# hritikbharucha/Custom_Porechop_ABI

Measured on AMD Instinct MI355X. Metric: reads/sec trimmed (100k ONT reads x 50 adapter pairs), higher is better.
Workload: dtype int32

## Files before the change

custom_porechop_abi_amd/csrc/pcabi_dp.h:

```cpp
#pragma once

#ifndef PCABI_ROW_FENCE
#define PCABI_ROW_FENCE 1
#endif
#ifndef PCABI_TAB_PD
#define PCABI_TAB_PD 0
#endif
#ifndef PCABI_TAB_PD_LONG
#define PCABI_TAB_PD_LONG 1
#endif

#include <stdint.h>
#include <algorithm>

#ifdef __HIPCC__
#define PCABI_HD __host__ __device__ __forceinline__
#else
#define PCABI_HD inline
#endif

namespace pcabi {

constexpr int NEG = -(1 << 28);

// ... 892 lines not shown
PCABI_HD bool shift_ok(int L, int rpl, const Scoring &s, int &P, int &B) {
    for (int p = shift_pmax(rpl); p >= 2; p >>= 1) {
        int blo, bhi;
        if (shift_range(L, rpl, s, p, blo, bhi)) {
            P = p;
            B = (blo + bhi) / 2;
            return true;
        }
    }
    return false;
}

PCABI_HD bool packed_ok(int L, int rpl, const Scoring &s) {
    switch (rpl) {
#define PCABI_PK(R) case R: return packed_ok_t<R>(L, s);
    PCABI_PK(4) PCABI_PK(8) PCABI_PK(12) PCABI_PK(16) PCABI_PK(20) PCABI_PK(24) PCABI_PK(28) PCABI_PK(32)
    PCABI_PK(36) PCABI_PK(40) PCABI_PK(44) PCABI_PK(48) PCABI_PK(52) PCABI_PK(56) PCABI_PK(60) PCABI_PK(64)
    PCABI_PK(68) PCABI_PK(72) PCABI_PK(76) PCABI_PK(80) PCABI_PK(84) PCABI_PK(88)
#undef PCABI_PK
    default: return false;
    }
}

template <int RPL, bool AFFINE, typename LAY = pk::Lay<RPL>, int PD = PCABI_TAB_PD>
struct LanePacked {
    using Y = LAY;
    int32_t G[RPL + 1];
    int32_t HK[RPL + 1];
    int bscore, bi, bj, blt, btrail, bprec;
    uint32_t battr;
    int slt_last, ht_last, hp_last;
    int32_t k_ge, k_go, k_gev, k_geh, neg2;
    int32_t k_gex, k_vo;
    int32_t bkey;

    template <typename TabRow, bool LAST, bool GATE = false>
    PCABI_HD void column(const TabRow &tab, const int j, const int L, const int off, const bool owned = true) {
        int32_t gup = Y::start(j + off) + k_go;
        int32_t vup = neg2;
        int slt_up = LT_NONE, vt_up = 0, vp_up = 0;
        int32_t lv = 0, lh = 0, ls = 0;
        int lslt = LT_D;
        bool lhext = false;
        constexpr int NQ = RPL / 4;
        int32_t t[RPL + 2];
        if (PD > 0) {
// ... 388 lines not shown
    const int np = (n - 1) / 4;
    uint32_t cur = tr(0), nx = tr(1);
    int j = 1;
#pragma unroll 1
    for (int q = 0; q < np; ++q, j += 4) {
        const uint32_t w = cur;
        cur = nx;
        nx = tr(q + 2);
        ls.advance();
        ls.template column<decltype(tabfn(0))>(tabfn((int)(w & 0xFFu)), j, off);
        ls.step();
        ls.template column<decltype(tabfn(0))>(tabfn((int)((w >> 8) & 0xFFu)), j + 1, off);
        ls.step();
        ls.template column<decltype(tabfn(0))>(tabfn((int)((w >> 16) & 0xFFu)), j + 2, off);
        ls.step();
        ls.template column<decltype(tabfn(0))>(tabfn((int)(w >> 24)), j + 3, off);
    }
#pragma unroll 1
    for (; j < n; ++j) {
        ls.advance();
        ls.template column<decltype(tabfn(0))>(tabfn((int)((cur >> (8 * ((j - 1) & 3))) & 0xFFu)), j, off);
    }
    return shift_last<RPL, PD>(ls, tabfn((int)((cur >> (8 * ((n - 1) & 3))) & 0xFFu)), n, L, sc);
}

template <int RPL, bool AFFINE, bool CHUNK = false, typename ReadFn, typename TabFn0, typename TabFn1>
PCABI_HD Result align_lane_packed_long(ReadFn &rd0, ReadFn &rd1, int n, const TabFn0 &tab0, const TabFn1 &tab1,
                                       int L, const Scoring sc, int own_lo = 1, int own_hi = -1) {
    int n_fin;
    Best b = packed_best<RPL, AFFINE, CHUNK, pk::LayL<RPL, 0>, PCABI_TAB_PD_LONG>(rd0, n, tab0, L, sc, own_lo, own_hi,
                                                                                 n_fin);
    const Best bm = packed_best<RPL, AFFINE, CHUNK, pk::LayL<RPL, 1>, PCABI_TAB_PD_LONG>(rd1, n, tab1, L, sc, own_lo,
                                                                                        own_hi, n_fin);
    b.attr |= bm.attr;
    return finish(b, L, n_fin);
}

struct SplitIn {
    int32_t gup, vup;
    int slt, vt, vp;
    int score, bi, lt, trail, prec;
    uint32_t attr;
};

template <int R, bool AFFINE, typename LAY>
struct LaneSplit {
// ... 352 lines not shown
```

custom_porechop_abi_amd/csrc/pcabi_engine.hip:

```cpp
#include <hip/hip_runtime.h>

#include <algorithm>
#include <atomic>
#include <cstdio>
#include <cstdlib>
#include <cstring>
#include <mutex>
#include <string>
#include <thread>
#include <vector>

#include "../../include/pcabi.h"
#include "pcabi_dp.h"
#include "pcabi_kern.h"
#include "pcabi_host.h"

namespace {
thread_local std::string g_err;
}

namespace pcabi_eng {
int fail(int code, const std::string &msg) {
    g_err = msg;
    return code;
// ... 327 lines not shown
        dispatch_fast(d.rpl, d.kind == GENERIC, p, affine, grid, st);
    return 0;
}

bool bucket_packed_ok(int b, const std::vector<int32_t> &lens, const pcabi::Scoring &sc) {
    if (kBuckets[b].kind == WIDE || kBuckets[b].kind == LONG) return true;
    if (kBuckets[b].kind != FAST || kBuckets[b].rpl > pcabi::pk::MAX_RPL) return false;
    for (int32_t L : lens)
        if (!pcabi::packed_ok(L, kBuckets[b].rpl, sc)) return false;
    return true;
}

int bucket_pack_mode(int b, const std::vector<int32_t> &lens, const pcabi::Scoring &sc) {
    if (!bucket_packed_ok(b, lens, sc)) return 0;
    if (kBuckets[b].kind != FAST || kBuckets[b].rpl > 32) return 1;
    for (int32_t L : lens)
        if (!pcabi::layt_ok(L, kBuckets[b].rpl, sc)) return 1;
    return 2;
}


void bucket_shift(int b, const std::vector<int32_t> &lens, const pcabi::Scoring &sc, int pack_mode, KParams &p) {
    p.shift_p = p.shift_b = 0;
    if (pack_mode != 2 || lens.empty() || sc.go == sc.ge) return;
    const char *e = std::getenv("PCABI_SHIFT");
    if (e && e[0] == '0') return;
    const int rpl = kBuckets[b].rpl;
    for (int P = pcabi::shift_pmax(rpl); P >= 2; P >>= 1) {
        int lo = INT32_MIN, hi = INT32_MAX;
        bool ok = true;
        for (int32_t L : lens) {
            int blo, bhi;
            if (!pcabi::shift_range(L, rpl, sc, P, blo, bhi)) { ok = false; break; }
            lo = std::max(lo, blo);
            hi = std::min(hi, bhi);
        }
        if (ok && lo <= hi) {
            p.shift_p = P;
            p.shift_b = lo + (hi - lo) / 2;
            return;
        }
    }
}

}

namespace {

constexpr int kMaxFastBuckets = 4;

// ... 660 lines not shown
```

custom_porechop_abi_amd/csrc/pcabi_k_group.hip:

```cpp
#include "pcabi_kern.h"

namespace pcabi_eng {

template <int CLS>
__global__ __launch_bounds__(256) void k_align_group(GroupParams gp) {
    constexpr int MAXR = group_max_rpl(CLS);
    __shared__ __attribute__((aligned(16))) int32_t tab[4 * kTabW * MAXR];
    int32_t *wave_tab = tab + (threadIdx.x >> 6) * kTabW * MAXR;
    const int64_t b = blockIdx.x;
    int s = 0;
    while (s + 1 < gp.n_seg && b >= gp.seg[s + 1].block0) ++s;
    const GroupSeg &g = gp.seg[s];
    KParams p{};
    p.tiles = g.tiles;
    p.tile_off = g.tile_off;
    p.win_len = g.win_len;
    p.n_win = g.n_win;
    p.adp_pad = g.adp_pad;
    p.adp_len = g.adp_len;
    p.adp_id = g.adp_id;
    p.n_adp = g.n_adp;
    p.out = g.out;
    p.out_stride = g.out_stride;
    p.sc = gp.sc;
    p.shift_p = g.shift_p;
    p.shift_b = g.shift_b;
    const int64_t lb = b - g.block0;
    if constexpr (CLS == 0) {
        if (g.shift_p > 0) {
            switch (g.rpl) {
#define T(R) case R: cross_block<R, true, SHIFT>(p, lb, wave_tab); break;
            T(4) T(8) T(12) T(16) T(20) T(24) T(28) T(32)
#undef T
            }
        } else {
            switch (g.rpl) {
#define T(R) case R: cross_block<R, true, TAGGED>(p, lb, wave_tab); break;
            T(4) T(8) T(12) T(16) T(20) T(24) T(28) T(32)
#undef T
            }
        }
    } else {
        switch (g.rpl) {
#define P(R) case R: cross_block<R, true, PACKED>(p, lb, wave_tab); break;
        P(36) P(40) P(44) P(48) P(52) P(56) P(60) P(64)
#undef P
        }
    }
}

void dispatch_group(int cls, const GroupParams &p, int64_t blocks, hipStream_t st) {
    if (blocks <= 0) return;
    if (cls == 0) hipLaunchKernelGGL((k_align_group<0>), dim3((unsigned)blocks), dim3(256), 0, st, p);
    else hipLaunchKernelGGL((k_align_group<1>), dim3((unsigned)blocks), dim3(256), 0, st, p);
}

}
```

custom_porechop_abi_amd/csrc/pcabi_k_packed_large.hip:

```cpp
#include "pcabi_kern.h"

namespace pcabi_eng {

void dispatch_packed_large(int rpl, bool long_kind, const KParams &p, bool affine, dim3 grid, hipStream_t st) {
    if (long_kind) {
        switch (rpl) {
        case 96: launch<96, LONG>(p, affine, grid, st); break;
        case 112: launch<112, LONG>(p, affine, grid, st); break;
        case 128: launch<128, LONG>(p, affine, grid, st); break;
        }
        return;
    }
    switch (rpl) {
#define C(R) case R: launch<R, PACKED>(p, affine, grid, st); break;
    C(36) C(40) C(44) C(48) C(52) C(56) C(60) C(64) C(68) C(72) C(76) C(80) C(84) C(88)
#undef C
    }
}

}
```

custom_porechop_abi_amd/csrc/pcabi_kern.h:

```cpp
#pragma once
#include <hip/hip_runtime.h>

#include <algorithm>
#include <cstdint>
#include <cstdlib>
#include <string>
#include <type_traits>

#include "../../include/pcabi.h"
#include "pcabi_dp.h"

#ifndef PCABI_WAVES
#define PCABI_WAVES 1
#endif

void pcabi_poison(void *p, size_t bytes);
void pcabi_poison_async(void *p, size_t bytes, hipStream_t st);

namespace pcabi_eng {

int fail(int code, const std::string &msg);

#define HIP_TRY(expr)                                                                   \
    do {                                                                                \
        hipError_t e_ = (expr);                                                         \
        if (e_ != hipSuccess)                                                           \
            return fail(PCABI_E_DEVICE, std::string(#expr) + ": " + hipGetErrorString(e_)); \
    } while (0)

enum Kind { FAST = 0, GENERIC = 1, PACKED = 2, WIDE = 3, LONG = 4, STRIPED = 5,
            TAGGED = 6,
            SHIFT = 7 };
struct BucketDef {
    int rpl;
    Kind kind;
};
constexpr BucketDef kBuckets[] = {
    {4, FAST},  {8, FAST},  {12, FAST}, {16, FAST}, {20, FAST}, {24, FAST}, {28, FAST}, {32, FAST},
    {36, FAST}, {40, FAST}, {44, FAST}, {48, FAST}, {52, FAST}, {56, FAST}, {60, FAST}, {64, FAST},
    {68, WIDE}, {72, WIDE}, {76, WIDE}, {80, WIDE}, {84, WIDE}, {88, WIDE},
    {96, LONG}, {112, LONG}, {128, LONG},
    {16, GENERIC}, {32, GENERIC}, {64, GENERIC}, {96, GENERIC}, {128, GENERIC},
    {256, STRIPED}};
constexpr int kNumBuckets = sizeof(kBuckets) / sizeof(kBuckets[0]);
constexpr int kStripedBucket = kNumBuckets - 1;
constexpr int kMaxRPL = 128;
constexpr int kStripeRows = 32;
constexpr int kStripeTab = 64;

struct KParams {
    const uint8_t *codes;
    const int64_t *win_off;
    const int32_t *win_len;
    int64_t n_win;
    const uint32_t *tiles;
// ... 86 lines not shown
    for (int e = lane; e < kTabW * RPL; e += 64) {
        const int c = e / RPL, srow = e % RPL + 1;
        const uint32_t *ap = p.adp_pad + (int64_t)a_local * (RPL / 4);
        auto code = [&](int sl) { return (int)((ap[(sl - 1) / 4] >> (8 * ((sl - 1) & 3))) & 0xFFu); };
        wave_tab[e] = pcabi::pk::sub_key<RPL, decltype(code), Y>(srow, c, code, off, p.sc);
    }
    __syncthreads();
}

template <int RPL>
__device__ __forceinline__ void fill_wave_tab_shift(const KParams &p, int a_local, int L, int32_t *wave_tab) {
    const int off = RPL - L;
    const int lane = threadIdx.x & 63;
    for (int e = lane; e < kTabW * RPL; e += 64) {
        const int c = e / RPL, srow = e % RPL + 1;
        const uint32_t *ap = p.adp_pad + (int64_t)a_local * (RPL / 4);
        auto code = [&](int sl) { return (int)((ap[(sl - 1) / 4] >> (8 * ((sl - 1) & 3))) & 0xFFu); };
        wave_tab[e] = pcabi::pk::sub_key_shift<RPL>(srow, c, code, off, p.sc);
    }
    __syncthreads();
}

template <int RPL>
__device__ __forceinline__ void fill_wave_tab_long(const KParams &p, int a_local, int L, int32_t *wave_tab) {
    const int off = RPL - L;
    const int lane = threadIdx.x & 63;
    const uint32_t *ap = p.adp_pad + (int64_t)a_local * (RPL / 4);
    auto code = [&](int sl) { return (int)((ap[(sl - 1) / 4] >> (8 * ((sl - 1) & 3))) & 0xFFu); };
    for (int e = lane; e < kTabW * RPL; e += 64) {
        const int c = e / RPL, srow = e % RPL + 1;
        wave_tab[e] = pcabi::pk::sub_key<RPL, decltype(code), pcabi::pk::LayL<RPL, 0>>(srow, c, code, off, p.sc);
        wave_tab[kTabW * RPL + e] =
            pcabi::pk::sub_key<RPL, decltype(code), pcabi::pk::LayL<RPL, 1>>(srow, c, code, off, p.sc);
    }
    __syncthreads();
}

constexpr int kShift4MaxRows = 24;

template <int RPL, bool AFFINE, int KIND>
__device__ __forceinline__ void run_lane(const KParams &p, int a_local, int64_t w, int64_t out_idx,
                                         int32_t *wave_tab, int64_t tile_off) {
    AdapterRegs<RPL> adp;
    if constexpr (KIND != LONG) adp.load(p.adp_pad + (int64_t)a_local * (RPL / 4));
    const int L = __builtin_amdgcn_readfirstlane(p.adp_len[a_local]);
    if constexpr (KIND == PACKED) fill_wave_tab<RPL>(p, a_local, L, wave_tab);
    if constexpr (KIND == TAGGED) fill_wave_tab<RPL, pcabi::pk::LayT<RPL>>(p, a_local, L, wave_tab);
    if constexpr (KIND == SHIFT) fill_wave_tab_shift<RPL>(p, a_local, L, wave_tab);
    if constexpr (KIND == LONG) fill_wave_tab_long<RPL>(p, a_local, L, wave_tab);
    if (w < 0) return;
    const int n = p.win_len[w];
    pcabi::Result r;
    bool uniform = false;
    if constexpr (KIND == SHIFT) {
        const int n0 = __builtin_amdgcn_readfirstlane(n);
        const int P = __builtin_amdgcn_readfirstlane(p.shift_p);
        if (RPL <= kShift4MaxRows && n0 > 0 && (P & 3) == 0 && __builtin_amdgcn_ballot_w64(n != n0 || tile_off < 0) == 0) {
            const uint32_t *base = p.tiles + tile_off + (threadIdx.x & 255);
            auto tr = [&](int q) { return base[(int64_t)q * 256]; };
            auto tabfn = [&](int rc) { return LdsRow{wave_tab + rc * RPL}; };
            r = pcabi::align_lane_shift4<RPL>(tr, n0, tabfn, L, p.sc, P, p.shift_b);
            uniform = true;
        }
    }
    if (uniform) {
    } else if (n <= 0) {
        r = empty_result();
    } else {
        WindowReader rd = tile_off >= 0
            ? WindowReader(p.tiles + tile_off + (threadIdx.x & 255), 256, 0)
            : [&] {
                  const uint8_t *b = p.codes + p.win_off[w];
                  const int a0 = (int)((uintptr_t)b & 3);
                  return WindowReader(reinterpret_cast<const uint32_t *>(b - a0), 1, 8 * a0);
              }();
        if constexpr (KIND == PACKED) {
            auto tabfn = [&](int rc) { return LdsRow{wave_tab + rc * RPL}; };
            r = pcabi::align_lane_packed<(RPL <= pcabi::pk::MAX_RPL ? RPL : 4), AFFINE>(rd, n, tabfn, L, p.sc);
        } else if constexpr (KIND == TAGGED) {
            static_assert(RPL <= 32 && AFFINE, "run-tagged layout: affine buckets of <= 32 rows");
            auto tabfn = [&](int rc) { return LdsRow{wave_tab + rc * RPL}; };
            r = pcabi::align_lane_packed<RPL, true, false, pcabi::pk::LayT<RPL>>(rd, n, tabfn, L, p.sc);
        } else if constexpr (KIND == SHIFT) {
            static_assert(RPL <= 32 && AFFINE, "gap-extend frame: affine buckets of <= 32 rows");
            auto tabfn = [&](int rc) { return LdsRow{wave_tab + rc * RPL}; };
            r = pcabi::align_lane_shift<RPL>(rd, n, tabfn, L, p.sc, p.shift_p, p.shift_b);
        } else if constexpr (KIND == LONG) {
            WindowReader rd1 = rd;
            auto tab0 = [&](int rc) { return LdsRow{wave_tab + rc * RPL}; };
            auto tab1 = [&](int rc) { return LdsRow{wave_tab + kTabW * RPL + rc * RPL}; };
            r = pcabi::align_lane_packed_long<RPL, AFFINE>(rd, rd1, n, tab0, tab1, L, p.sc);
        } else if constexpr (KIND == FAST) {
            r = pcabi::align_lane_fast<RPL, AFFINE>(rd, n, adp, L, p.sc);
        } else {
            r = pcabi::align_lane_generic<RPL, AFFINE>(rd, n, adp, L, p.sc);
        }
    }
    if (p.compat) {
        int en_match = 0;
        if (r.rs >= 0 && r.diag_en && r.l1 > 0) {
            const uint8_t *ab = reinterpret_cast<const uint8_t *>(p.adp_pad + (int64_t)a_local * (RPL / 4));
            en_match = p.codes[p.win_off[w] + r.re] == ab[RPL - L + r.ae];
        }
        p.compat[out_idx] = pcabi::compat_flag(r, n, en_match);
        return;
    }
    store_result(p.out, p.out_stride, out_idx, r);
}

template <int KIND, int RPL>
constexpr int wave_tab_ints() {
    return (KIND == PACKED || KIND == TAGGED || KIND == SHIFT) ? kTabW * RPL : (KIND == LONG ? 2 * kTabW * RPL : 1);
}

template <int RPL, bool AFFINE, int KIND>
__device__ __forceinline__ void cross_block(const KParams &p, int64_t b, int32_t *wave_tab) {
    const int64_t k = b >> 3;
    const int a_local = (int)(k % p.n_adp);
    const int64_t tile = (k / p.n_adp) * 8 + (b & 7);
    const int64_t w = tile * 256 + threadIdx.x;
    const int a_glob = p.adp_id[a_local];
    const int64_t toff = w < p.n_win ? p.tile_off[tile] : 0;
    run_lane<RPL, AFFINE, KIND>(p, a_local, w < p.n_win ? w : -1, (int64_t)a_glob * p.n_win + w, wave_tab, toff);
}

template <int RPL, bool AFFINE, int KIND>
__global__ __launch_bounds__(256, PCABI_WAVES) void k_align(KParams p) {
    __shared__ __attribute__((aligned(16))) int32_t tab[4 * wave_tab_ints<KIND, RPL>()];
    int32_t *wave_tab = tab + (threadIdx.x >> 6) * wave_tab_ints<KIND, RPL>();
    if (p.task_win == nullptr) {
        cross_block<RPL, AFFINE, KIND>(p, blockIdx.x, wave_tab);
    } else {
        int64_t wave = (int64_t)blockIdx.x * 4 + (threadIdx.x >> 6);
        const bool live = wave < p.n_waves;
        if (!live) wave = p.n_waves - 1;
// ... 441 lines not shown
```

Measured before the change: 16.83 million.

## Add packed gap-extend shifted frame kernel for 36-64 row affine buckets

```diff
diff --git a/custom_porechop_abi_amd/csrc/pcabi_dp.h b/custom_porechop_abi_amd/csrc/pcabi_dp.h
--- a/custom_porechop_abi_amd/csrc/pcabi_dp.h
+++ b/custom_porechop_abi_amd/csrc/pcabi_dp.h
@@ -938,6 +938,54 @@
     }
 }
 
+constexpr int PSHIFT_PMAX = 512;
+PCABI_HD bool pshift_range(int L, int rpl, const Scoring &s, int P, int &blo, int &bhi) {
+    if (rpl < 36 || rpl > 64 || s.go == s.ge || !packed_ok(L, rpl, s)) return false;
+    if (P < 2 || P > PSHIFT_PMAX) return false;
+    const int e = -s.ge, bs = best_sub(s) > 0 ? best_sub(s) : 0;
+    int msub = s.mi < s.ma ? s.mi : s.ma;
+    if (msub > 0) msub = 0;
+    const int off = rpl - L;
+    int lo0 = s.go, hi0 = s.go + e + e * (P - 1);
+    for (int sl = 1; sl <= rpl; ++sl) {
+        const int i = sl - off;
+        const int slo = i >= 1 ? s.go + (i - 1) * s.ge : 0, shi = i >= 1 ? i * bs : 0;
+        const int ulo = i >= 2 ? s.go + (i - 2) * s.ge : 0, uhi = i >= 2 ? (i - 1) * bs : 0;
+        int lo = slo + s.go;
+        if (ulo + msub < lo) lo = ulo + msub;
+        int hi = shi + (s.go + e > 0 ? s.go + e : 0);
+        if (uhi + bs > hi) hi = uhi + bs;
+        lo += e * (sl - 1);
+        hi += e * (sl + P - 1);
+        if (lo < lo0) lo0 = lo;
+        if (hi > hi0) hi0 = hi;
+    }
+    blo = hi0 - 511;
+    bhi = lo0 + 511;
+    return blo <= bhi;
+}
+PCABI_HD bool pshift_bucket(const int32_t *lens, int n_adp, int rpl, const Scoring &s, int &P, int &B) {
+    if (n_adp < 1) return false;
+    for (int p = PSHIFT_PMAX; p >= 2; p >>= 1) {
+        int lo = -(1 << 30), hi = 1 << 30;
+        bool ok = true;
+        for (int k = 0; k < n_adp && ok; ++k) {
+            int blo, bhi;
+            ok = pshift_range(lens[k], rpl, s, p, blo, bhi);
+            if (ok) {
+                lo = blo > lo ? blo : lo;
+                hi = bhi < hi ? bhi : hi;
+            }
+        }
+        if (ok && lo <= hi) {
+            P = p;
+            B = lo + (hi - lo) / 2;
+            return true;
+        }
+    }
+    return false;
+}
+
 template <int RPL, bool AFFINE, typename LAY = pk::Lay<RPL>, int PD = PCABI_TAB_PD>
 struct LanePacked {
     using Y = LAY;
@@ -1372,6 +1420,153 @@
         ls.template column<decltype(tabfn(0))>(tabfn((int)((cur >> (8 * ((j - 1) & 3))) & 0xFFu)), j, off);
     }
     return shift_last<RPL, PD>(ls, tabfn((int)((cur >> (8 * ((n - 1) & 3))) & 0xFFu)), n, L, sc);
+}
+
+namespace pk {
+template <int RPL, typename AdpFn>
+PCABI_HD int32_t sub_key_pshift(int s, int c, const AdpFn &adp, int off, const Scoring &sc) {
+    using Y = Lay<RPL>;
+    const int d = -sc.go - sc.ge;
+    if (s <= off) return Y::TB3 + Y::sc(d);
+    return (c == adp(s)) ? (Y::sc(sc.ma + d) + Y::TB3 + Y::INC_M) : (Y::sc(sc.mi + d) + Y::TB3 + Y::INC_D);
+}
+constexpr int32_t PSENT = (int32_t)0x80000000;
+}
+
+template <int RPL, int PD = PCABI_TAB_PD>
+struct LanePShift {
+    using Y = pk::Lay<RPL>;
+    LanePacked<RPL, true, Y, PD> st;
+    int32_t kgo;
+    int32_t ftop;
+    int32_t k_e;
+    int32_t k_eR;
+    int32_t k_rb;
+    int jj, P;
+
+    PCABI_HD void init(int L, const Scoring &sc, int P_, int B) {
+        using pk::addw;
+        const int off = RPL - L;
+        P = P_;
+        jj = 0;
+        k_e = Y::sc(-sc.ge);
+        k_eR = Y::sc(-sc.ge * RPL);
+        k_rb = Y::sc(sc.ge * P);
+        ftop = Y::sc(-B);
+        kgo = Y::sc(sc.go - sc.ge);
+        int32_t fs = vreg(addw(ftop, kgo));
+#pragma unroll
+        for (int s = 1; s <= RPL; ++s) {
+            fs = addw(fs, k_e);
+            st.G[s] = addw(Y::start(off - s), fs);
+            st.HK[s] = addw(fs, Y::sc(-1)) | Y::TB1;
+        }
+        st.bkey = Y::start(-L);
+        st.bj = 0;
+    }
+
+    PCABI_HD void advance() {
+        using pk::addw;
+        ++jj;
+        ftop = addw(ftop, k_e);
+        if (jj == P) {
+#pragma unroll
+            for (int s = 1; s <= RPL; ++s) {
+                st.G[s] = addw(st.G[s], k_rb);
+                st.HK[s] = addw(st.HK[s], k_rb);
+            }
+            jj = 0;
+            ftop = addw(ftop, k_rb);
+        }
+    }
+
+    template <typename TabRow>
+    PCABI_HD void column(const TabRow &tab, const int j, const int off) {
+        using pk::addw;
+        const int32_t kg = vreg(kgo);
+        const int32_t top = addw(ftop, kgo);
+        int32_t gup = addw(Y::start(j + off), top);
+        int32_t vup = pk::PSENT;
+        int32_t diag = addw(addw(Y::start(j - 1 + off), top), pk::negw(k_e));
+        constexpr int NQ = RPL / 4;
+        int32_t t[RPL + 2];
+        if (PD > 0) {
+#pragma unroll
+            for (int q = 0; q <= PD && q < NQ; ++q) tab.quad(q, t + 4 * q + 1);
+        }
+        diag = addw(diag, PD > 0 ? t[1] : tab(1));
+        int32_t lv = 0, ls = 0;
+#pragma unroll
+        for (int s = 1; s <= RPL; ++s) {
+            if (PD > 0 && (s & 3) == 1) {
+                const int q = (s - 1) / 4 + PD + 1;
+                if (q < NQ) tab.quad(q, t + 4 * q + 1);
+            }
+            int32_t diag_nx = 0;
+            if (s < RPL) diag_nx = st.G[s] + (PD > 0 ? t[s + 1] : tab(s + 1));
+            const int32_t hn = std::max(st.HK[s], st.G[s]);
+            const int32_t vn2 = std::max(vup, gup) | Y::TB2;
+            const int32_t sn = max3i(diag, vn2, hn);
+            if (s == RPL) { lv = vn2; ls = sn; }
+            st.G[s] = (sn & ~Y::TBM) + kg;
+            st.HK[s] = hn | Y::TB1;
+            gup = st.G[s];
+            vup = vn2;
+            diag = diag_nx;
+#if defined(__HIP_DEVICE_COMPILE__)
+            if (PCABI_ROW_FENCE > 0 && (s % (PCABI_ROW_FENCE > 0 ? PCABI_ROW_FENCE : 1)) == 0) __builtin_amdgcn_sched_barrier(0);
+#endif
+        }
+        const int32_t corr = addw(std::max(lv | Y::TB3, ls & ~Y::TBM), pk::negw(addw(ftop, k_eR)));
+        const bool upd = corr > (st.bkey | ((1 << Y::SC_SH) - 1));
+        st.bkey = upd ? corr : st.bkey;
+        st.bj = upd ? j : st.bj;
+    }
+
+    PCABI_HD void to_lay(const Scoring &sc) {
+        using pk::addw;
+        using pk::negw;
+        int32_t ch = vreg(negw(ftop));
+        int32_t cg = addw(ch, Y::sc(sc.ge));
+#pragma unroll
+        for (int s = 1; s <= RPL; ++s) {
+            cg = addw(cg, negw(k_e));
+            ch = addw(ch, negw(k_e));
+            st.G[s] = addw(st.G[s], cg);
+            st.HK[s] = addw(st.HK[s], ch);
+        }
+    }
+};
+
+template <int RPL, int PD = PCABI_TAB_PD, typename ReadFn, typename TabFn>
+PCABI_HD Result align_lane_pshift(ReadFn &rd, int n, const TabFn &tabfn, int L, const Scoring sc, int P, int B) {
+    using Y = pk::Lay<RPL>;
+    LanePShift<RPL, PD> ls;
+    const int off = RPL - L;
+    ls.init(L, sc, P, B);
+    int r = rd(1);
+#pragma unroll 1
+    for (int j = 1; j < n; ++j) {
+        const int rn = rd(j + 1);
+        ls.advance();
+        ls.template column<decltype(tabfn(r))>(tabfn(r), j, off);
+        r = rn;
+    }
+    ls.to_lay(sc);
+    auto &st = ls.st;
+    st.k_ge = Y::sc(sc.ge);
+    st.k_go = Y::sc(sc.go);
+    st.k_gev = st.k_geh = 0;
+    st.k_gex = st.k_ge;
+    st.k_vo = 0;
+    st.neg2 = Y::sc(pk::neg_score(sc)) | Y::TB2;
+    st.materialize(L);
+    const pk::ShiftRow<decltype(tabfn(r))> row{tabfn(r), Y::sc(sc.ge)};
+    st.template column<decltype(row), true>(row, n, L, off);
+    Best b;
+    b.score = st.bscore; b.bi = st.bi; b.bj = st.bj; b.attr = Y::to_std(st.battr, st.bj);
+    b.ltype = st.blt; b.trail = st.btrail; b.precd = st.bprec;
+    return finish(b, L, n);
 }
 
 template <int RPL, bool AFFINE, bool CHUNK = false, typename ReadFn, typename TabFn0, typename TabFn1>
diff --git a/custom_porechop_abi_amd/csrc/pcabi_engine.hip b/custom_porechop_abi_amd/csrc/pcabi_engine.hip
--- a/custom_porechop_abi_amd/csrc/pcabi_engine.hip
+++ b/custom_porechop_abi_amd/csrc/pcabi_engine.hip
@@ -373,10 +373,19 @@
 
 void bucket_shift(int b, const std::vector<int32_t> &lens, const pcabi::Scoring &sc, int pack_mode, KParams &p) {
     p.shift_p = p.shift_b = 0;
-    if (pack_mode != 2 || lens.empty() || sc.go == sc.ge) return;
+    if (lens.empty() || sc.go == sc.ge) return;
     const char *e = std::getenv("PCABI_SHIFT");
     if (e && e[0] == '0') return;
     const int rpl = kBuckets[b].rpl;
+    if (pack_mode == 1 && kBuckets[b].kind == FAST && rpl >= 36 && rpl <= 64) {
+        int P, B;
+        if (pcabi::pshift_bucket(lens.data(), (int)lens.size(), rpl, sc, P, B)) {
+            p.shift_p = P;
+            p.shift_b = B;
+        }
+        return;
+    }
+    if (pack_mode != 2) return;
     for (int P = pcabi::shift_pmax(rpl); P >= 2; P >>= 1) {
         int lo = INT32_MIN, hi = INT32_MAX;
         bool ok = true;
diff --git a/custom_porechop_abi_amd/csrc/pcabi_k_group.hip b/custom_porechop_abi_amd/csrc/pcabi_k_group.hip
--- a/custom_porechop_abi_amd/csrc/pcabi_k_group.hip
+++ b/custom_porechop_abi_amd/csrc/pcabi_k_group.hip
@@ -41,10 +41,18 @@
             }
         }
     } else {
-        switch (g.rpl) {
+        if (g.shift_p > 0) {
+            switch (g.rpl) {
+#define P(R) case R: cross_block<R, true, PSHIFT>(p, lb, wave_tab); break;
+            P(36) P(40) P(44) P(48) P(52) P(56) P(60) P(64)
+#undef P
+            }
+        } else {
+            switch (g.rpl) {
 #define P(R) case R: cross_block<R, true, PACKED>(p, lb, wave_tab); break;
-        P(36) P(40) P(44) P(48) P(52) P(56) P(60) P(64)
+            P(36) P(40) P(44) P(48) P(52) P(56) P(60) P(64)
 #undef P
+            }
         }
     }
 }
diff --git a/custom_porechop_abi_amd/csrc/pcabi_k_packed_large.hip b/custom_porechop_abi_amd/csrc/pcabi_k_packed_large.hip
--- a/custom_porechop_abi_amd/csrc/pcabi_k_packed_large.hip
+++ b/custom_porechop_abi_amd/csrc/pcabi_k_packed_large.hip
@@ -11,6 +11,13 @@
         }
         return;
     }
+    if (affine && p.shift_p > 0 && !p.task_win) {
+        switch (rpl) {
+#define S(R) case R: hipLaunchKernelGGL((k_align<R, true, PSHIFT>), grid, dim3(256), 0, st, p); return;
+        S(36) S(40) S(44) S(48) S(52) S(56) S(60) S(64)
+#undef S
+        }
+    }
     switch (rpl) {
 #define C(R) case R: launch<R, PACKED>(p, affine, grid, st); break;
     C(36) C(40) C(44) C(48) C(52) C(56) C(60) C(64) C(68) C(72) C(76) C(80) C(84) C(88)
diff --git a/custom_porechop_abi_amd/csrc/pcabi_kern.h b/custom_porechop_abi_amd/csrc/pcabi_kern.h
--- a/custom_porechop_abi_amd/csrc/pcabi_kern.h
+++ b/custom_porechop_abi_amd/csrc/pcabi_kern.h
@@ -30,7 +30,8 @@
 
 enum Kind { FAST = 0, GENERIC = 1, PACKED = 2, WIDE = 3, LONG = 4, STRIPED = 5,
             TAGGED = 6,
-            SHIFT = 7 };
+            SHIFT = 7,
+            PSHIFT = 8 };
 struct BucketDef {
     int rpl;
     Kind kind;
@@ -163,6 +164,19 @@
 }
 
 template <int RPL>
+__device__ __forceinline__ void fill_wave_tab_pshift(const KParams &p, int a_local, int L, int32_t *wave_tab) {
+    const int off = RPL - L;
+    const int lane = threadIdx.x & 63;
+    for (int e = lane; e < kTabW * RPL; e += 64) {
+        const int c = e / RPL, srow = e % RPL + 1;
+        const uint32_t *ap = p.adp_pad + (int64_t)a_local * (RPL / 4);
+        auto code = [&](int sl) { return (int)((ap[(sl - 1) / 4] >> (8 * ((sl - 1) & 3))) & 0xFFu); };
+        wave_tab[e] = pcabi::pk::sub_key_pshift<RPL>(srow, c, code, off, p.sc);
+    }
+    __syncthreads();
+}
+
+template <int RPL>
 __device__ __forceinline__ void fill_wave_tab_long(const KParams &p, int a_local, int L, int32_t *wave_tab) {
     const int off = RPL - L;
     const int lane = threadIdx.x & 63;
@@ -188,6 +202,7 @@
     if constexpr (KIND == PACKED) fill_wave_tab<RPL>(p, a_local, L, wave_tab);
     if constexpr (KIND == TAGGED) fill_wave_tab<RPL, pcabi::pk::LayT<RPL>>(p, a_local, L, wave_tab);
     if constexpr (KIND == SHIFT) fill_wave_tab_shift<RPL>(p, a_local, L, wave_tab);
+    if constexpr (KIND == PSHIFT) fill_wave_tab_pshift<RPL>(p, a_local, L, wave_tab);
     if constexpr (KIND == LONG) fill_wave_tab_long<RPL>(p, a_local, L, wave_tab);
     if (w < 0) return;
     const int n = p.win_len[w];
@@ -226,6 +241,10 @@
             static_assert(RPL <= 32 && AFFINE, "gap-extend frame: affine buckets of <= 32 rows");
             auto tabfn = [&](int rc) { return LdsRow{wave_tab + rc * RPL}; };
             r = pcabi::align_lane_shift<RPL>(rd, n, tabfn, L, p.sc, p.shift_p, p.shift_b);
+        } else if constexpr (KIND == PSHIFT) {
+            static_assert(RPL >= 36 && RPL <= 64 && AFFINE, "packed gap-extend frame: affine buckets of 36..64 rows");
+            auto tabfn = [&](int rc) { return LdsRow{wave_tab + rc * RPL}; };
+            r = pcabi::align_lane_pshift<RPL>(rd, n, tabfn, L, p.sc, p.shift_p, p.shift_b);
         } else if constexpr (KIND == LONG) {
             WindowReader rd1 = rd;
             auto tab0 = [&](int rc) { return LdsRow{wave_tab + rc * RPL}; };
@@ -251,7 +270,7 @@
 
 template <int KIND, int RPL>
 constexpr int wave_tab_ints() {
-    return (KIND == PACKED || KIND == TAGGED || KIND == SHIFT) ? kTabW * RPL : (KIND == LONG ? 2 * kTabW * RPL : 1);
+    return (KIND == PACKED || KIND == TAGGED || KIND == SHIFT || KIND == PSHIFT) ? kTabW * RPL : (KIND == LONG ? 2 * kTabW * RPL : 1);
 }
 
 template <int RPL, bool AFFINE, int KIND>
diff --git a/profiles/r09/k_align_group1_pshift64_inner_column.s b/profiles/r09/k_align_group1_pshift64_inner_column.s
--- /dev/null
+++ b/profiles/r09/k_align_group1_pshift64_inner_column.s
@@ -0,0 +1,670 @@
+.LBB1_985:
+	s_and_b32 s0, s51, 24
+	v_mov_b32_e32 v143, v11
+	s_waitcnt vmcnt(1)
+	v_lshrrev_b64 v[10:11], s0, v[8:9]
+	v_lshl_add_u32 v11, v142, 8, v12
+	v_mov_b32_e32 v142, v141
+	ds_read_b64 v[146:147], v11
+	s_add_i32 s54, s50, 0xfff01000
+	s_and_b32 s55, s50, 0xff000
+	s_add_i32 s53, s45, s46
+	s_and_b32 s54, s54, 0xff000
+	s_sub_i32 s55, s55, s43
+	s_add_i32 s54, s53, s54
+	s_add_i32 s55, s55, s53
+	s_waitcnt lgkmcnt(0)
+	v_add_u32_e32 v144, s55, v146
+	v_max_i32_e32 v108, v108, v105
+	s_bitset1_b32 s54, 21
+	v_add_u32_e32 v146, v147, v105
+	v_max3_i32 v105, v144, s54, v108
+	v_and_b32_e32 v105, 0xffcfffff, v105
+	v_add_u32_e32 v105, v105, v142
+	v_or_b32_e32 v108, 0x100000, v108
+	s_add_i32 s0, s47, 1
+	ds_read_b32 v144, v11 offset:8
+	v_max_i32_e32 v147, s54, v105
+	v_max_i32_e32 v139, v139, v140
+	v_or_b32_e32 v147, 0x200000, v147
+	v_max3_i32 v146, v146, v147, v139
+	s_waitcnt lgkmcnt(0)
+	v_add_u32_e32 v144, v144, v140
+	v_and_b32_e32 v140, 0xffcfffff, v146
+	v_add_u32_e32 v140, v140, v142
+	v_or_b32_e32 v139, 0x100000, v139
+	ds_read_b32 v146, v11 offset:12
+	v_max_i32_e32 v147, v147, v140
+	v_max_i32_e32 v138, v138, v137
+	v_or_b32_e32 v147, 0x200000, v147
+	v_max3_i32 v144, v144, v147, v138
+	s_waitcnt lgkmcnt(0)
+	v_add_u32_e32 v146, v146, v137
+	v_and_b32_e32 v137, 0xffcfffff, v144
+	v_add_u32_e32 v137, v137, v142
+	v_or_b32_e32 v138, 0x100000, v138
+	ds_read_b32 v144, v11 offset:16
+	v_max_i32_e32 v147, v147, v137
+	v_max_i32_e32 v136, v136, v135
+	v_or_b32_e32 v147, 0x200000, v147
+	v_max3_i32 v146, v146, v147, v136
+	s_waitcnt lgkmcnt(0)
+	v_add_u32_e32 v144, v144, v135
+	v_and_b32_e32 v135, 0xffcfffff, v146
+	v_add_u32_e32 v135, v135, v142
+	v_or_b32_e32 v136, 0x100000, v136
+	ds_read_b32 v146, v11 offset:20
+	v_max_i32_e32 v147, v147, v135
+	v_max_i32_e32 v134, v134, v133
+	v_or_b32_e32 v147, 0x200000, v147
+	v_max3_i32 v144, v144, v147, v134
+	s_waitcnt lgkmcnt(0)
+	v_add_u32_e32 v146, v146, v133
+	v_and_b32_e32 v133, 0xffcfffff, v144
+	v_add_u32_e32 v133, v133, v142
+	v_or_b32_e32 v134, 0x100000, v134
+	ds_read_b32 v144, v11 offset:24
+	v_max_i32_e32 v147, v147, v133
+	v_max_i32_e32 v132, v132, v131
+	v_or_b32_e32 v147, 0x200000, v147
+	v_max3_i32 v146, v146, v147, v132
+	s_waitcnt lgkmcnt(0)
+	v_add_u32_e32 v144, v144, v131
+	v_and_b32_e32 v131, 0xffcfffff, v146
+	v_add_u32_e32 v131, v131, v142
+	v_or_b32_e32 v132, 0x100000, v132
+	ds_read_b32 v146, v11 offset:28
+	v_max_i32_e32 v147, v147, v131
+	v_max_i32_e32 v130, v130, v129
+	v_or_b32_e32 v147, 0x200000, v147
+	v_max3_i32 v144, v144, v147, v130
+	s_waitcnt lgkmcnt(0)
+	v_add_u32_e32 v146, v146, v129
+	v_and_b32_e32 v129, 0xffcfffff, v144
+	v_add_u32_e32 v129, v129, v142
+	v_or_b32_e32 v130, 0x100000, v130
+	ds_read_b32 v144, v11 offset:32
+	v_max_i32_e32 v147, v147, v129
+	v_max_i32_e32 v128, v128, v127
+	v_or_b32_e32 v147, 0x200000, v147
+	v_max3_i32 v146, v146, v147, v128
+	s_waitcnt lgkmcnt(0)
+	v_add_u32_e32 v144, v144, v127
+	v_and_b32_e32 v127, 0xffcfffff, v146
+	v_add_u32_e32 v127, v127, v142
+	v_or_b32_e32 v128, 0x100000, v128
+	ds_read_b32 v146, v11 offset:36
+	v_max_i32_e32 v147, v147, v127
+	v_max_i32_e32 v126, v126, v125
+	v_or_b32_e32 v147, 0x200000, v147
+	v_max3_i32 v144, v144, v147, v126
+	s_waitcnt lgkmcnt(0)
+	v_add_u32_e32 v146, v146, v125
+	v_and_b32_e32 v125, 0xffcfffff, v144
+	v_add_u32_e32 v125, v125, v142
+	v_or_b32_e32 v126, 0x100000, v126
+	ds_read_b32 v144, v11 offset:40
+	v_max_i32_e32 v147, v147, v125
+	v_max_i32_e32 v124, v124, v123
+	v_or_b32_e32 v147, 0x200000, v147
+	v_max3_i32 v146, v146, v147, v124
+	s_waitcnt lgkmcnt(0)
+	v_add_u32_e32 v144, v144, v123
+	v_and_b32_e32 v123, 0xffcfffff, v146
+	v_add_u32_e32 v123, v123, v142
+	v_or_b32_e32 v124, 0x100000, v124
+	ds_read_b32 v146, v11 offset:44
+	v_max_i32_e32 v147, v147, v123
+	v_max_i32_e32 v122, v122, v121
+	v_or_b32_e32 v147, 0x200000, v147
+	v_max3_i32 v144, v144, v147, v122
+	s_waitcnt lgkmcnt(0)
+	v_add_u32_e32 v146, v146, v121
+	v_and_b32_e32 v121, 0xffcfffff, v144
+	v_add_u32_e32 v121, v121, v142
+	v_or_b32_e32 v122, 0x100000, v122
+	ds_read_b32 v144, v11 offset:48
+	v_max_i32_e32 v147, v147, v121
+	v_max_i32_e32 v120, v120, v119
+	v_or_b32_e32 v147, 0x200000, v147
+	v_max3_i32 v146, v146, v147, v120
+	s_waitcnt lgkmcnt(0)
+	v_add_u32_e32 v144, v144, v119
+	v_and_b32_e32 v119, 0xffcfffff, v146
+	v_add_u32_e32 v119, v119, v142
+	v_or_b32_e32 v120, 0x100000, v120
+	ds_read_b32 v146, v11 offset:52
+	v_max_i32_e32 v147, v147, v119
+	v_max_i32_e32 v118, v118, v117
+	v_or_b32_e32 v147, 0x200000, v147
+	v_max3_i32 v144, v144, v147, v118
+	s_waitcnt lgkmcnt(0)
+	v_add_u32_e32 v146, v146, v117
+	v_and_b32_e32 v117, 0xffcfffff, v144
+	v_add_u32_e32 v117, v117, v142
+	v_or_b32_e32 v118, 0x100000, v118
+	ds_read_b32 v144, v11 offset:56
+	v_max_i32_e32 v147, v147, v117
+	v_max_i32_e32 v116, v116, v115
+	v_or_b32_e32 v147, 0x200000, v147
+	v_max3_i32 v146, v146, v147, v116
+	s_waitcnt lgkmcnt(0)
+	v_add_u32_e32 v144, v144, v115
+	v_and_b32_e32 v115, 0xffcfffff, v146
+	v_add_u32_e32 v115, v115, v142
+	v_or_b32_e32 v116, 0x100000, v116
+	ds_read_b32 v146, v11 offset:60
+	v_max_i32_e32 v147, v147, v115
+	v_max_i32_e32 v114, v114, v113
+	v_or_b32_e32 v147, 0x200000, v147
+	v_max3_i32 v144, v144, v147, v114
+	s_waitcnt lgkmcnt(0)
+	v_add_u32_e32 v146, v146, v113
+	v_and_b32_e32 v113, 0xffcfffff, v144
+	v_add_u32_e32 v113, v113, v142
+	v_or_b32_e32 v114, 0x100000, v114
+	ds_read_b32 v144, v11 offset:64
+	v_max_i32_e32 v147, v147, v113
+	v_max_i32_e32 v112, v112, v111
+	v_or_b32_e32 v147, 0x200000, v147
+	v_max3_i32 v146, v146, v147, v112
+	s_waitcnt lgkmcnt(0)
+	v_add_u32_e32 v144, v144, v111
+	v_and_b32_e32 v111, 0xffcfffff, v146
+	v_add_u32_e32 v111, v111, v142
+	v_or_b32_e32 v112, 0x100000, v112
+	ds_read_b32 v146, v11 offset:68
+	v_max_i32_e32 v147, v147, v111
+	v_max_i32_e32 v110, v110, v109
+	v_or_b32_e32 v147, 0x200000, v147
+	v_max3_i32 v144, v144, v147, v110
+	s_waitcnt lgkmcnt(0)
+	v_add_u32_e32 v146, v146, v109
+	v_and_b32_e32 v109, 0xffcfffff, v144
+	v_add_u32_e32 v109, v109, v142
+	v_or_b32_e32 v110, 0x100000, v110
+	ds_read_b32 v144, v11 offset:72
+	v_max_i32_e32 v147, v147, v109
+	v_max_i32_e32 v107, v107, v106
+	v_or_b32_e32 v147, 0x200000, v147
+	v_max3_i32 v146, v146, v147, v107
+	s_waitcnt lgkmcnt(0)
+	v_add_u32_e32 v144, v144, v106
+	v_and_b32_e32 v106, 0xffcfffff, v146
+	v_add_u32_e32 v106, v106, v142
+	v_or_b32_e32 v107, 0x100000, v107
+	ds_read_b32 v146, v11 offset:76
+	v_max_i32_e32 v147, v147, v106
+	v_max_i32_e32 v104, v104, v103
+	v_or_b32_e32 v147, 0x200000, v147
+	v_max3_i32 v144, v144, v147, v104
+	s_waitcnt lgkmcnt(0)
+	v_add_u32_e32 v146, v146, v103
+	v_and_b32_e32 v103, 0xffcfffff, v144
+	v_add_u32_e32 v103, v103, v142
+	v_or_b32_e32 v104, 0x100000, v104
+	ds_read_b32 v144, v11 offset:80
+	v_max_i32_e32 v147, v147, v103
+	v_max_i32_e32 v102, v102, v101
+	v_or_b32_e32 v147, 0x200000, v147
+	v_max3_i32 v146, v146, v147, v102
+	s_waitcnt lgkmcnt(0)
+	v_add_u32_e32 v144, v144, v101
+	v_and_b32_e32 v101, 0xffcfffff, v146
+	v_add_u32_e32 v101, v101, v142
+	v_or_b32_e32 v102, 0x100000, v102
+	ds_read_b32 v146, v11 offset:84
+	v_max_i32_e32 v147, v147, v101
+	v_max_i32_e32 v100, v100, v99
+	v_or_b32_e32 v147, 0x200000, v147
+	v_max3_i32 v144, v144, v147, v100
+	s_waitcnt lgkmcnt(0)
+	v_add_u32_e32 v146, v146, v99
+	v_and_b32_e32 v99, 0xffcfffff, v144
+	v_add_u32_e32 v99, v99, v142
+	v_or_b32_e32 v100, 0x100000, v100
+	ds_read_b32 v144, v11 offset:88
+	v_max_i32_e32 v147, v147, v99
+	v_max_i32_e32 v98, v98, v97
+	v_or_b32_e32 v147, 0x200000, v147
+	v_max3_i32 v146, v146, v147, v98
+	s_waitcnt lgkmcnt(0)
+	v_add_u32_e32 v144, v144, v97
+	v_and_b32_e32 v97, 0xffcfffff, v146
+	v_add_u32_e32 v97, v97, v142
+	v_or_b32_e32 v98, 0x100000, v98
+	ds_read_b32 v146, v11 offset:92
+	v_max_i32_e32 v147, v147, v97
+	v_max_i32_e32 v96, v96, v95
+	v_or_b32_e32 v147, 0x200000, v147
+	v_max3_i32 v144, v144, v147, v96
+	s_waitcnt lgkmcnt(0)
+	v_add_u32_e32 v146, v146, v95
+	v_and_b32_e32 v95, 0xffcfffff, v144
+	v_add_u32_e32 v95, v95, v142
+	v_or_b32_e32 v96, 0x100000, v96
+	ds_read_b32 v144, v11 offset:96
+	v_max_i32_e32 v147, v147, v95
+	v_max_i32_e32 v94, v94, v93
+	v_or_b32_e32 v147, 0x200000, v147
+	v_max3_i32 v146, v146, v147, v94
+	s_waitcnt lgkmcnt(0)
+	v_add_u32_e32 v144, v144, v93
+	v_and_b32_e32 v93, 0xffcfffff, v146
+	v_add_u32_e32 v93, v93, v142
+	v_or_b32_e32 v94, 0x100000, v94
+	ds_read_b32 v146, v11 offset:100
+	v_max_i32_e32 v147, v147, v93
+	v_max_i32_e32 v92, v92, v91
+	v_or_b32_e32 v147, 0x200000, v147
+	v_max3_i32 v144, v144, v147, v92
+	s_waitcnt lgkmcnt(0)
+	v_add_u32_e32 v146, v146, v91
+	v_and_b32_e32 v91, 0xffcfffff, v144
+	v_add_u32_e32 v91, v91, v142
+	v_or_b32_e32 v92, 0x100000, v92
+	ds_read_b32 v144, v11 offset:104
+	v_max_i32_e32 v147, v147, v91
+	v_max_i32_e32 v90, v90, v89
+	v_or_b32_e32 v147, 0x200000, v147
+	v_max3_i32 v146, v146, v147, v90
+	s_waitcnt lgkmcnt(0)
+	v_add_u32_e32 v144, v144, v89
+	v_and_b32_e32 v89, 0xffcfffff, v146
+	v_add_u32_e32 v89, v89, v142
+	v_or_b32_e32 v90, 0x100000, v90
+	ds_read_b32 v146, v11 offset:108
+	v_max_i32_e32 v147, v147, v89
+	v_max_i32_e32 v88, v88, v87
+	v_or_b32_e32 v147, 0x200000, v147
+	v_max3_i32 v144, v144, v147, v88
+	s_waitcnt lgkmcnt(0)
+	v_add_u32_e32 v146, v146, v87
+	v_and_b32_e32 v87, 0xffcfffff, v144
+	v_add_u32_e32 v87, v87, v142
+	v_or_b32_e32 v88, 0x100000, v88
+	ds_read_b32 v144, v11 offset:112
+	v_max_i32_e32 v147, v147, v87
+	v_max_i32_e32 v86, v86, v85
+	v_or_b32_e32 v147, 0x200000, v147
+	v_max3_i32 v146, v146, v147, v86
+	s_waitcnt lgkmcnt(0)
+	v_add_u32_e32 v144, v144, v85
+	v_and_b32_e32 v85, 0xffcfffff, v146
+	v_add_u32_e32 v85, v85, v142
+	v_or_b32_e32 v86, 0x100000, v86
+	ds_read_b32 v146, v11 offset:116
+	v_max_i32_e32 v147, v147, v85
+	v_max_i32_e32 v84, v84, v83
+	v_or_b32_e32 v147, 0x200000, v147
+	v_max3_i32 v144, v144, v147, v84
+	s_waitcnt lgkmcnt(0)
+	v_add_u32_e32 v146, v146, v83
+	v_and_b32_e32 v83, 0xffcfffff, v144
+	v_add_u32_e32 v83, v83, v142
+	v_or_b32_e32 v84, 0x100000, v84
+	ds_read_b32 v144, v11 offset:120
+	v_max_i32_e32 v147, v147, v83
+	v_max_i32_e32 v82, v82, v81
+	v_or_b32_e32 v147, 0x200000, v147
+	v_max3_i32 v146, v146, v147, v82
+	s_waitcnt lgkmcnt(0)
+	v_add_u32_e32 v144, v144, v81
+	v_and_b32_e32 v81, 0xffcfffff, v146
+	v_add_u32_e32 v81, v81, v142
+	v_or_b32_e32 v82, 0x100000, v82
+	ds_read_b32 v146, v11 offset:124
+	v_max_i32_e32 v147, v147, v81
+	v_max_i32_e32 v80, v80, v79
+	v_or_b32_e32 v147, 0x200000, v147
+	v_max3_i32 v144, v144, v147, v80
+	s_waitcnt lgkmcnt(0)
+	v_add_u32_e32 v146, v146, v79
+	v_and_b32_e32 v79, 0xffcfffff, v144
+	v_add_u32_e32 v79, v79, v142
+	v_or_b32_e32 v80, 0x100000, v80
+	ds_read_b32 v144, v11 offset:128
+	v_max_i32_e32 v147, v147, v79
+	v_max_i32_e32 v78, v78, v77
+	v_or_b32_e32 v147, 0x200000, v147
+	v_max3_i32 v146, v146, v147, v78
+	s_waitcnt lgkmcnt(0)
+	v_add_u32_e32 v144, v144, v77
+	v_and_b32_e32 v77, 0xffcfffff, v146
+	v_add_u32_e32 v77, v77, v142
+	v_or_b32_e32 v78, 0x100000, v78
+	ds_read_b32 v146, v11 offset:132
+	v_max_i32_e32 v147, v147, v77
+	v_max_i32_e32 v76, v76, v75
+	v_or_b32_e32 v147, 0x200000, v147
+	v_max3_i32 v144, v144, v147, v76
+	s_waitcnt lgkmcnt(0)
+	v_add_u32_e32 v146, v146, v75
+	v_and_b32_e32 v75, 0xffcfffff, v144
+	v_add_u32_e32 v75, v75, v142
+	v_or_b32_e32 v76, 0x100000, v76
+	ds_read_b32 v144, v11 offset:136
+	v_max_i32_e32 v147, v147, v75
+	v_max_i32_e32 v74, v74, v73
+	v_or_b32_e32 v147, 0x200000, v147
+	v_max3_i32 v146, v146, v147, v74
+	s_waitcnt lgkmcnt(0)
+	v_add_u32_e32 v144, v144, v73
+	v_and_b32_e32 v73, 0xffcfffff, v146
+	v_add_u32_e32 v73, v73, v142
+	v_or_b32_e32 v74, 0x100000, v74
+	ds_read_b32 v146, v11 offset:140
+	v_max_i32_e32 v147, v147, v73
+	v_max_i32_e32 v72, v72, v71
+	v_or_b32_e32 v147, 0x200000, v147
+	v_max3_i32 v144, v144, v147, v72
+	s_waitcnt lgkmcnt(0)
+	v_add_u32_e32 v146, v146, v71
+	v_and_b32_e32 v71, 0xffcfffff, v144
+	v_add_u32_e32 v71, v71, v142
+	v_or_b32_e32 v72, 0x100000, v72
+	ds_read_b32 v144, v11 offset:144
+	v_max_i32_e32 v147, v147, v71
+	v_max_i32_e32 v70, v70, v69
+	v_or_b32_e32 v147, 0x200000, v147
+	v_max3_i32 v146, v146, v147, v70
+	s_waitcnt lgkmcnt(0)
+	v_add_u32_e32 v144, v144, v69
+	v_and_b32_e32 v69, 0xffcfffff, v146
+	v_add_u32_e32 v69, v69, v142
+	v_or_b32_e32 v70, 0x100000, v70
+	ds_read_b32 v146, v11 offset:148
+	v_max_i32_e32 v147, v147, v69
+	v_max_i32_e32 v68, v68, v67
+	v_or_b32_e32 v147, 0x200000, v147
+	v_max3_i32 v144, v144, v147, v68
+	s_waitcnt lgkmcnt(0)
+	v_add_u32_e32 v146, v146, v67
+	v_and_b32_e32 v67, 0xffcfffff, v144
+	v_add_u32_e32 v67, v67, v142
+	v_or_b32_e32 v68, 0x100000, v68
+	ds_read_b32 v144, v11 offset:152
+	v_max_i32_e32 v147, v147, v67
+	v_max_i32_e32 v66, v66, v65
+	v_or_b32_e32 v147, 0x200000, v147
+	v_max3_i32 v146, v146, v147, v66
+	s_waitcnt lgkmcnt(0)
+	v_add_u32_e32 v144, v144, v65
+	v_and_b32_e32 v65, 0xffcfffff, v146
+	v_add_u32_e32 v65, v65, v142
+	v_or_b32_e32 v66, 0x100000, v66
+	ds_read_b32 v146, v11 offset:156
+	v_max_i32_e32 v147, v147, v65
+	v_max_i32_e32 v64, v64, v63
+	v_or_b32_e32 v147, 0x200000, v147
+	v_max3_i32 v144, v144, v147, v64
+	s_waitcnt lgkmcnt(0)
+	v_add_u32_e32 v146, v146, v63
+	v_and_b32_e32 v63, 0xffcfffff, v144
+	v_add_u32_e32 v63, v63, v142
+	v_or_b32_e32 v64, 0x100000, v64
+	ds_read_b32 v144, v11 offset:160
+	v_max_i32_e32 v147, v147, v63
+	v_max_i32_e32 v62, v62, v61
+	v_or_b32_e32 v147, 0x200000, v147
+	v_max3_i32 v146, v146, v147, v62
+	s_waitcnt lgkmcnt(0)
+	v_add_u32_e32 v144, v144, v61
+	v_and_b32_e32 v61, 0xffcfffff, v146
+	v_add_u32_e32 v61, v61, v142
+	v_or_b32_e32 v62, 0x100000, v62
+	ds_read_b32 v146, v11 offset:164
+	v_max_i32_e32 v147, v147, v61
+	v_max_i32_e32 v60, v60, v59
+	v_or_b32_e32 v147, 0x200000, v147
+	v_max3_i32 v144, v144, v147, v60
+	s_waitcnt lgkmcnt(0)
+	v_add_u32_e32 v146, v146, v59
+	v_and_b32_e32 v59, 0xffcfffff, v144
+	v_add_u32_e32 v59, v59, v142
+	v_or_b32_e32 v60, 0x100000, v60
+	ds_read_b32 v144, v11 offset:168
+	v_max_i32_e32 v147, v147, v59
+	v_max_i32_e32 v58, v58, v57
+	v_or_b32_e32 v147, 0x200000, v147
+	v_max3_i32 v146, v146, v147, v58
+	s_waitcnt lgkmcnt(0)
+	v_add_u32_e32 v144, v144, v57
+	v_and_b32_e32 v57, 0xffcfffff, v146
+	v_add_u32_e32 v57, v57, v142
+	v_or_b32_e32 v58, 0x100000, v58
+	ds_read_b32 v146, v11 offset:172
+	v_max_i32_e32 v147, v147, v57
+	v_max_i32_e32 v56, v56, v55
+	v_or_b32_e32 v147, 0x200000, v147
+	v_max3_i32 v144, v144, v147, v56
+	s_waitcnt lgkmcnt(0)
+	v_add_u32_e32 v146, v146, v55
+	v_and_b32_e32 v55, 0xffcfffff, v144
+	v_add_u32_e32 v55, v55, v142
+	v_or_b32_e32 v56, 0x100000, v56
+	ds_read_b32 v144, v11 offset:176
+	v_max_i32_e32 v147, v147, v55
+	v_max_i32_e32 v54, v54, v53
+	v_or_b32_e32 v147, 0x200000, v147
+	v_max3_i32 v146, v146, v147, v54
+	s_waitcnt lgkmcnt(0)
+	v_add_u32_e32 v144, v144, v53
+	v_and_b32_e32 v53, 0xffcfffff, v146
+	v_add_u32_e32 v53, v53, v142
+	v_or_b32_e32 v54, 0x100000, v54
+	ds_read_b32 v146, v11 offset:180
+	v_max_i32_e32 v147, v147, v53
+	v_max_i32_e32 v52, v52, v51
+	v_or_b32_e32 v147, 0x200000, v147
+	v_max3_i32 v144, v144, v147, v52
+	s_waitcnt lgkmcnt(0)
+	v_add_u32_e32 v146, v146, v51
+	v_and_b32_e32 v51, 0xffcfffff, v144
+	v_add_u32_e32 v51, v51, v142
+	v_or_b32_e32 v52, 0x100000, v52
+	ds_read_b32 v144, v11 offset:184
+	v_max_i32_e32 v147, v147, v51
+	v_max_i32_e32 v50, v50, v49
+	v_or_b32_e32 v147, 0x200000, v147
+	v_max3_i32 v146, v146, v147, v50
+	s_waitcnt lgkmcnt(0)
+	v_add_u32_e32 v144, v144, v49
+	v_and_b32_e32 v49, 0xffcfffff, v146
+	v_add_u32_e32 v49, v49, v142
+	v_or_b32_e32 v50, 0x100000, v50
+	ds_read_b32 v146, v11 offset:188
+	v_max_i32_e32 v147, v147, v49
+	v_max_i32_e32 v48, v48, v47
+	v_or_b32_e32 v147, 0x200000, v147
+	v_max3_i32 v144, v144, v147, v48
+	s_waitcnt lgkmcnt(0)
+	v_add_u32_e32 v146, v146, v47
+	v_and_b32_e32 v47, 0xffcfffff, v144
+	v_add_u32_e32 v47, v47, v142
+	v_or_b32_e32 v48, 0x100000, v48
+	ds_read_b32 v144, v11 offset:192
+	v_max_i32_e32 v147, v147, v47
+	v_max_i32_e32 v46, v46, v45
+	v_or_b32_e32 v147, 0x200000, v147
+	v_max3_i32 v146, v146, v147, v46
+	s_waitcnt lgkmcnt(0)
+	v_add_u32_e32 v144, v144, v45
+	v_and_b32_e32 v45, 0xffcfffff, v146
+	v_add_u32_e32 v45, v45, v142
+	v_or_b32_e32 v46, 0x100000, v46
+	ds_read_b32 v146, v11 offset:196
+	v_max_i32_e32 v147, v147, v45
+	v_max_i32_e32 v44, v44, v43
+	v_or_b32_e32 v147, 0x200000, v147
+	v_max3_i32 v144, v144, v147, v44
+	s_waitcnt lgkmcnt(0)
+	v_add_u32_e32 v146, v146, v43
+	v_and_b32_e32 v43, 0xffcfffff, v144
+	v_add_u32_e32 v43, v43, v142
+	v_or_b32_e32 v44, 0x100000, v44
+	ds_read_b32 v144, v11 offset:200
+	v_max_i32_e32 v147, v147, v43
+	v_max_i32_e32 v42, v42, v41
+	v_or_b32_e32 v147, 0x200000, v147
+	v_max3_i32 v146, v146, v147, v42
+	s_waitcnt lgkmcnt(0)
+	v_add_u32_e32 v144, v144, v41
+	v_and_b32_e32 v41, 0xffcfffff, v146
+	v_add_u32_e32 v41, v41, v142
+	v_or_b32_e32 v42, 0x100000, v42
+	ds_read_b32 v146, v11 offset:204
+	v_max_i32_e32 v147, v147, v41
+	v_max_i32_e32 v40, v40, v39
+	v_or_b32_e32 v147, 0x200000, v147
+	v_max3_i32 v144, v144, v147, v40
+	s_waitcnt lgkmcnt(0)
+	v_add_u32_e32 v146, v146, v39
+	v_and_b32_e32 v39, 0xffcfffff, v144
+	v_add_u32_e32 v39, v39, v142
+	v_or_b32_e32 v40, 0x100000, v40
+	ds_read_b32 v144, v11 offset:208
+	v_max_i32_e32 v147, v147, v39
+	v_max_i32_e32 v38, v38, v37
+	v_or_b32_e32 v147, 0x200000, v147
+	v_max3_i32 v146, v146, v147, v38
+	s_waitcnt lgkmcnt(0)
+	v_add_u32_e32 v144, v144, v37
+	v_and_b32_e32 v37, 0xffcfffff, v146
+	v_add_u32_e32 v37, v37, v142
+	v_or_b32_e32 v38, 0x100000, v38
+	ds_read_b32 v146, v11 offset:212
+	v_max_i32_e32 v147, v147, v37
+	v_max_i32_e32 v36, v36, v35
+	v_or_b32_e32 v147, 0x200000, v147
+	v_max3_i32 v144, v144, v147, v36
+	s_waitcnt lgkmcnt(0)
+	v_add_u32_e32 v146, v146, v35
+	v_and_b32_e32 v35, 0xffcfffff, v144
+	v_add_u32_e32 v35, v35, v142
+	v_or_b32_e32 v36, 0x100000, v36
+	ds_read_b32 v144, v11 offset:216
+	v_max_i32_e32 v147, v147, v35
+	v_max_i32_e32 v34, v34, v33
+	v_or_b32_e32 v147, 0x200000, v147
+	v_max3_i32 v146, v146, v147, v34
+	s_waitcnt lgkmcnt(0)
+	v_add_u32_e32 v144, v144, v33
+	v_and_b32_e32 v33, 0xffcfffff, v146
+	v_add_u32_e32 v33, v33, v142
+	v_or_b32_e32 v34, 0x100000, v34
+	ds_read_b32 v146, v11 offset:220
+	v_max_i32_e32 v147, v147, v33
+	v_max_i32_e32 v32, v32, v31
+	v_or_b32_e32 v147, 0x200000, v147
+	v_max3_i32 v144, v144, v147, v32
+	s_waitcnt lgkmcnt(0)
+	v_add_u32_e32 v146, v146, v31
+	v_and_b32_e32 v31, 0xffcfffff, v144
+	v_add_u32_e32 v31, v31, v142
+	v_or_b32_e32 v32, 0x100000, v32
+	ds_read_b32 v144, v11 offset:224
+	v_max_i32_e32 v147, v147, v31
+	v_max_i32_e32 v30, v30, v29
+	v_or_b32_e32 v147, 0x200000, v147
+	v_max3_i32 v146, v146, v147, v30
+	s_waitcnt lgkmcnt(0)
+	v_add_u32_e32 v144, v144, v29
+	v_and_b32_e32 v29, 0xffcfffff, v146
+	v_add_u32_e32 v29, v29, v142
+	v_or_b32_e32 v30, 0x100000, v30
+	ds_read_b32 v146, v11 offset:228
+	v_max_i32_e32 v147, v147, v29
+	v_max_i32_e32 v27, v27, v26
+	v_or_b32_e32 v147, 0x200000, v147
+	v_max3_i32 v144, v144, v147, v27
+	s_waitcnt lgkmcnt(0)
+	v_add_u32_e32 v146, v146, v26
+	v_and_b32_e32 v26, 0xffcfffff, v144
+	v_add_u32_e32 v26, v26, v142
+	v_or_b32_e32 v27, 0x100000, v27
+	ds_read_b32 v144, v11 offset:232
+	v_max_i32_e32 v147, v147, v26
+	v_max_i32_e32 v25, v25, v24
+	v_or_b32_e32 v147, 0x200000, v147
+	v_max3_i32 v146, v146, v147, v25
+	s_waitcnt lgkmcnt(0)
+	v_add_u32_e32 v144, v144, v24
+	v_and_b32_e32 v24, 0xffcfffff, v146
+	v_add_u32_e32 v24, v24, v142
+	v_or_b32_e32 v25, 0x100000, v25
+	ds_read_b32 v146, v11 offset:236
+	v_max_i32_e32 v147, v147, v24
+	v_max_i32_e32 v23, v23, v22
+	v_or_b32_e32 v147, 0x200000, v147
+	v_max3_i32 v144, v144, v147, v23
+	s_waitcnt lgkmcnt(0)
+	v_add_u32_e32 v146, v146, v22
+	v_and_b32_e32 v22, 0xffcfffff, v144
+	v_add_u32_e32 v22, v22, v142
+	v_or_b32_e32 v23, 0x100000, v23
+	ds_read_b32 v144, v11 offset:240
+	v_max_i32_e32 v147, v147, v22
+	v_max_i32_e32 v21, v21, v20
+	v_or_b32_e32 v147, 0x200000, v147
+	v_max3_i32 v146, v146, v147, v21
+	s_waitcnt lgkmcnt(0)
+	v_add_u32_e32 v144, v144, v20
+	v_and_b32_e32 v20, 0xffcfffff, v146
+	v_add_u32_e32 v20, v20, v142
+	v_or_b32_e32 v21, 0x100000, v21
+	ds_read_b32 v146, v11 offset:244
+	v_max_i32_e32 v147, v147, v20
+	v_max_i32_e32 v19, v19, v18
+	v_or_b32_e32 v147, 0x200000, v147
+	v_max3_i32 v144, v144, v147, v19
+	s_waitcnt lgkmcnt(0)
+	v_add_u32_e32 v146, v146, v18
+	v_and_b32_e32 v18, 0xffcfffff, v144
+	v_add_u32_e32 v18, v18, v142
+	v_or_b32_e32 v19, 0x100000, v19
+	ds_read_b32 v144, v11 offset:248
+	v_max_i32_e32 v147, v147, v18
+	v_max_i32_e32 v17, v17, v16
+	v_or_b32_e32 v147, 0x200000, v147
+	v_max3_i32 v146, v146, v147, v17
+	s_waitcnt lgkmcnt(0)
+	v_add_u32_e32 v144, v144, v16
+	v_and_b32_e32 v16, 0xffcfffff, v146
+	v_add_u32_e32 v16, v16, v142
+	v_or_b32_e32 v17, 0x100000, v17
+	ds_read_b32 v146, v11 offset:252
+	v_max_i32_e32 v11, v147, v16
+	v_max_i32_e32 v15, v15, v143
+	v_or_b32_e32 v147, 0x200000, v11
+	v_max3_i32 v11, v144, v147, v15
+	v_and_b32_e32 v11, 0xffcfffff, v11
+	v_add_u32_e32 v11, v11, v142
+	v_or_b32_e32 v15, 0x100000, v15
+	v_max_i32_e32 v144, v147, v11
+	s_waitcnt lgkmcnt(0)
+	v_add_u32_e32 v143, v146, v143
+	v_max_i32_e32 v4, v4, v14
+	v_or_b32_e32 v14, 0x200000, v144
+	v_max3_i32 v14, v143, v14, v4
+	v_and_b32_e32 v143, 0xffcfffff, v14
+	v_add_u32_e32 v14, v143, v142
+	v_or_b32_e32 v4, 0x100000, v4
+	v_or_b32_e32 v142, 0x300000, v144
+	v_max_i32_e32 v142, v142, v143
+	s_sub_i32 s53, s49, s45
+	v_add_u32_e32 v142, s53, v142
+	v_or_b32_e32 v143, 0x3fffff, v28
+	v_cmp_gt_i32_e32 vcc, v142, v143
+	s_addk_i32 s50, 0x1000
+	s_add_i32 s51, s51, 8
+	v_cndmask_b32_e32 v28, v28, v142, vcc
+	v_mov_b32_e32 v142, s47
+	v_cndmask_b32_e32 v5, v5, v142, vcc
+	v_cmp_eq_u32_e32 vcc, s0, v13
+	v_and_b32_e32 v142, 0xff, v10
+	s_or_b64 s[40:41], vcc, s[40:41]
+	v_mov_b32_e32 v10, s45
+	s_mov_b32 s47, s0
+	s_andn2_b64 exec, exec, s[40:41]
+	s_cbranch_execz .LBB1_1006
```

Result: faster. 17.24 million (median of 6 runs) (+2.4%).
